# cartographer-project/point_cloud_viewer

Measured on AMD Instinct MI355X. Metric: octree-build Mpoints/sec, higher is better.
Workload: dtype f64; 1 GPU; BASELINE config 2: 100 M Gaussian-cluster points (64 clusters, 1000 m cube, sigma 1-20 m), f64 SoA xyz + u8 rgb, resolution 1 mm, full build + LOD promotion; points_per_gpu=100000000, points_total=100000000, nodes=6073, parallelism=1 GPU

## Files before the change

point_cloud_viewer_amd/csrc/pcv_encode.hip:

```cpp
#include <algorithm>
#include <cstdlib>

#include "pcv_chain_dev.h"
#include "pcv_settle_dev.h"
#include "pcv_spec.h"

#ifndef PCV_KEEP_BRANCH
#define PCV_KEEP_BRANCH 0
#endif
#ifndef PCV_ENC_SEGMENTS
#define PCV_ENC_SEGMENTS 1
#endif

namespace {

__global__ __launch_bounds__(256) void leaf_encode_kernel(
    PcvLevels lv, const uint64_t* __restrict__ walk, uint64_t n, const double* __restrict__ x,
    const double* __restrict__ y, const double* __restrict__ z, PcvRouted routed, const uint8_t* __restrict__ color,
    uint32_t color_stride, const float* __restrict__ intensity, uint32_t* __restrict__ rank, uint4* __restrict__ payload,
    uint32_t* __restrict__ cx_hi, uint32_t* __restrict__ cy_hi, uint32_t* __restrict__ cz_hi,
    uint32_t* __restrict__ inten_bits) {
  const uint64_t i = (uint64_t)blockIdx.x * 256 + threadIdx.x;
  if (i >= n) return;
  uint64_t rec = walk[0];
// ... 355 lines not shown
                             : make_uint4((uint32_t)vx, (uint32_t)vy, (uint32_t)vz, rgb);
      }
    }
  }
  tid = wave * 64 + (int)pcv_lane_again();
  if (stage) {
    uint32_t rgb[2];
#pragma unroll
    for (int h = 0; h < 2; ++h) {
      const uint32_t t = (uint32_t)(h * BLOCK + tid);
      rgb[h] = (!(DIAG & 1) && t < here) ? pcv_load_rgb(color + (base + t) * color_stride, base + t + 1 < n) : 0u;
    }
    __syncthreads();
#pragma unroll
    for (int h = 0; h < 2; ++h) {
      const uint32_t t = (uint32_t)(h * BLOCK + tid);
      if (t < here) {
        const uint2 q = opay[t];
        __builtin_nontemporal_store(okey[t] | (rgb[h] >> 16), &rank[base + t]);
        __builtin_nontemporal_store(((uint64_t)(q.y | ((rgb[h] & 0xffffu) << 16)) << 32) | q.x, reinterpret_cast<uint64_t*>(payload) + base + t);
      }
    }
  }
  if (inten_bits) {
#pragma unroll
    for (int h = 0; h < 2; ++h) {
      const uint32_t t = (uint32_t)(h * BLOCK + tid);
      if (t < here) inten_bits[base + t] = __float_as_uint(intensity[base + t]);
    }
  }
}
#undef CP_WALK_GUARDED
#undef CP_WALK_TAME
#undef CP_CODE_LOOP
#undef CP_LOOP
#undef CP_BITS
#undef CP_KEEP_STEP
#undef CP_WALK_AT


constexpr int kHistBins = 16384;
constexpr int kHistBinsRows = 32768;
__global__ __launch_bounds__(1024) void rank_hist_kernel(const uint32_t* __restrict__ rank, uint64_t n, uint64_t chunk,
                                                          uint32_t bin_base, uint32_t nbins, uint32_t* __restrict__ counts,
                                                          int shift ,
                                                          uint32_t* __restrict__ rows ,
                                                          uint32_t row_stride) {
  extern __shared__ uint32_t hist[];
  for (uint32_t b = threadIdx.x; b < nbins; b += 1024) hist[b] = 0;
  __syncthreads();
  const uint64_t begin = (uint64_t)blockIdx.x * chunk;
  uint64_t end = begin + chunk;
  if (end > n) end = n;
  for (uint64_t i = begin + (uint64_t)threadIdx.x * 4; i < end; i += 4096) {
    if (i + 4 <= end) {
      const uint4 v = *reinterpret_cast<const uint4*>(rank + i);
      const uint32_t r[4] = {(v.x >> shift) - bin_base, (v.y >> shift) - bin_base, (v.z >> shift) - bin_base,
                             (v.w >> shift) - bin_base};
#pragma unroll
      for (int k = 0; k < 4; ++k)
        if (r[k] < nbins) atomicAdd(&hist[r[k]], 1u);
    } else {
      for (uint64_t j = i; j < end; ++j) {
        const uint32_t r = (rank[j] >> shift) - bin_base;
        if (r < nbins) atomicAdd(&hist[r], 1u);
      }
    }
  }
  __syncthreads();
  for (uint32_t b = threadIdx.x; b < nbins; b += 1024) {
    const uint32_t v = hist[b];
    if (v) atomicAdd(&counts[bin_base + b], v);
    if (rows) rows[(uint64_t)blockIdx.x * row_stride + bin_base + b] = v;
  }
}

struct alignas(16) PcvContRange {
  uint32_t from_level, to_level, pad0, pad1;
  double mn[3];
  double pad2;
};
static_assert(sizeof(PcvContRange) == 48, "continue range");
__device__ __forceinline__ void pcv_continue_codes(const PcvLevels& lv, const PcvContRange& rg, uint32_t& cx, uint32_t& cy, uint32_t& cz) {
  const int from = (int)rg.from_level, to = (int)rg.to_level;
  const uint32_t fe = lv.enc[from], te = lv.enc[to];
  double mx = rg.mn[0], my = rg.mn[1], mz = rg.mn[2];
  const double e = lv.edge[from];
  double px = pcv_decode_coord(fe, cx, mx, e), py = pcv_decode_coord(fe, cy, my, e), pz = pcv_decode_coord(fe, cz, mz, e);
  double vx = 0, vy = 0, vz = 0;
  for (int L = from + 1; L <= to; ++L)
    (void)pcv_chain_level<true>(lv.enc[L], lv.edge[L - 1], lv.edge[L], PcvRecip{lv.inv_edge[L], lv.inv_edge_lo[L]}, px, py, pz, mx, my,
                                mz, vx, vy, vz);
  cx = (uint32_t)pcv_val_to_code(te, vx);
  cy = (uint32_t)pcv_val_to_code(te, vy);
  cz = (uint32_t)pcv_val_to_code(te, vz);
}
template <bool kCompact>
__global__ __launch_bounds__(256) void spec_continue_kernel(PcvLevels lv, const PcvContRange* __restrict__ ranges,
                                                             const PcvSettleItem* __restrict__ items, uint4* __restrict__ payload,
                                                             uint4* __restrict__ wide ) {
  const PcvSettleItem it = items[blockIdx.x];
  const PcvContRange rg = ranges[it.rank];
  const uint32_t fe = lv.enc[rg.from_level], te = lv.enc[rg.to_level];
  uint2* __restrict__ pay2 = reinterpret_cast<uint2*>(payload);
  for (uint32_t s = it.begin + threadIdx.x; s < it.end; s += 256) {
    uint4 p = make_uint4(0, 0, 0, 0);
    uint2 q = make_uint2(0, 0);
// ... 472 lines not shown
```

point_cloud_viewer_amd/csrc/pcv_internal.h:

```cpp
#pragma once
#include <hip/hip_runtime.h>
#include <stdint.h>

#include <condition_variable>
#include <functional>
#include <map>
#include <mutex>
#include <string>
#include <thread>
#include <vector>

#include "../../include/pcv_hip.h"
#include "pcv_levels.h"
#include "pcv_sort_plan.h"
#include "pcv_spec.h"

#define PCV_HIP_CHECK(ctx, expr)                                                                   \
  do {                                                                                             \
    hipError_t _e = (expr);                                                                        \
    if (_e != hipSuccess) return (ctx)->fail(PCV_E_HIP, std::string(#expr) + ": " + hipGetErrorString(_e)); \
  } while (0)

struct PcvHostPool {
  std::vector<std::thread> threads;
// ... 343 lines not shown
  uint32_t* dst = nullptr;
  uint64_t n = 0, chunk = 0;
  int shift = 0, nbits = 0;
  const uint32_t *hist = nullptr, *totals = nullptr;
  const void* vec_in = nullptr;
  void* vec_out = nullptr;
  const uint32_t* plane_in = nullptr;
  uint32_t* plane_out = nullptr;
  const uint32_t* map = nullptr;
  uint32_t map_entries = 0;
  const void* ranges = nullptr;
  const uint32_t* order = nullptr;
  const uint8_t* color_in = nullptr;
  uint32_t color_stride = 3;
};
void pcv_sort_launch_rec12(pcv_ctx* ctx, const PcvSortRec12Args& a);
void pcv_sort_launch_scan(pcv_ctx* ctx, uint32_t* hist, int groups, uint32_t* totals);
void pcv_sort_generic_passes_u32(pcv_ctx* ctx, const PcvSortPlan& plan, int first, uint32_t* keys_a, uint32_t* keys_b,
                                 PcvSortPayload* payload, void* scratch, const uint32_t* map, uint32_t map_entries);

struct PcvNodeTableDev {
  uint32_t capacity;
  uint64_t* prefix;
  uint64_t* prefix_lo;
  uint32_t* lo;
  uint32_t* hi;
  uint32_t* parent;
  uint32_t* first_child;
  uint8_t* level;
  uint8_t* child_mask;
  uint8_t* open;
  uint32_t* bounds;
  uint32_t max_open = 0;
  uint32_t* counters;
};
struct PcvPackedNode {
  uint64_t prefix;
  uint32_t lo, hi, first_child;
  uint8_t level, child_mask, open, pad;
};
static_assert(sizeof(PcvPackedNode) == 24, "packed node");
constexpr size_t kPcvPackHeader = 256;
void pcv_launch_pack_node_table(pcv_ctx* ctx, const PcvNodeTableDev& t, void* packed );
size_t pcv_sample_count_scratch_words(uint32_t capacity, uint32_t max_open, int nlevels);
void pcv_launch_sample_tree_counts(pcv_ctx* ctx, const PcvNodeTableDev& t, const uint64_t* keys, uint32_t n, const PcvLevels& lv,
                                   double resolution, uint32_t max_points_per_node, uint32_t force_split_level1_mask, uint32_t* scratch,
                                   uint32_t saturate_above );
void pcv_launch_spec_tree(pcv_ctx* ctx, const PcvNodeTableDev& t, double upper, uint32_t force_mask, uint32_t* ord, uint32_t* walk,
                          uint32_t* sparent, uint8_t* slevel, uint32_t* info, uint32_t* pool_ctr );
int pcv_launch_spec_sample_tree(pcv_ctx* ctx, const uint64_t* sorted_keys, uint32_t ns, const PcvLevels& lv, double resolution, uint32_t thr,
                                double upper, uint32_t force_mask, uint64_t* list, uint32_t list_cap, uint32_t* ctr, uint32_t* walk,
                                uint32_t* sparent, uint8_t* slevel, uint32_t* info, uint32_t* pool_ctr);
void pcv_launch_spec_resolve(pcv_ctx* ctx, const PcvLevels& lv, double resolution, uint32_t cap, uint32_t force_mask, const uint32_t* walk,
                             const uint8_t* slevel, uint32_t tn, uint32_t* counts, uint32_t* nst, uint32_t* base, uint32_t* map,
                             uint32_t* out);
void pcv_launch_node_split(pcv_ctx* ctx, const PcvNodeTableDev& t, const void* sorted_keys, bool keys32, uint32_t n,
                           const PcvLevels& lv, double resolution, uint32_t max_points_per_node,
                           uint32_t force_split_level1_mask, const uint64_t* sorted_lo = nullptr);
void pcv_launch_chain_keys_deep(pcv_ctx* ctx, const PcvLevels& lv, uint64_t n, const double* x, const double* y,
                                const double* z, const PcvRouted& routed, uint32_t* const words[4]);
void pcv_launch_combine_words(pcv_ctx* ctx, uint64_t n, const uint32_t* const words[4], uint64_t* hi, uint64_t* lo);

struct PcvWalkTables {
  uint32_t num_nodes;
  const uint64_t* walk;
};
void pcv_launch_leaf_encode(pcv_ctx* ctx, const PcvLevels& lv, const PcvWalkTables& wt, uint64_t n, const double* x,
                            const double* y, const double* z, const PcvRouted& routed, const uint8_t* color,
                            uint32_t color_stride, const float* intensity, uint32_t* rank, void* payload ,
                            uint32_t* cx_hi,
                            uint32_t* cy_hi, uint32_t* cz_hi, uint32_t* inten_bits);

void pcv_launch_spec_encode(pcv_ctx* ctx, const PcvLevels& lv, const uint32_t* walk, uint64_t n, const double* x,
                            const double* y, const double* z, const PcvRouted& routed, const uint8_t* color,
                            uint32_t color_stride, const float* intensity, uint32_t* rank, void* payload ,
                            uint32_t* inten_bits, uint8_t* depth_grid, void* wide, uint32_t* pool_ctr, const uint32_t* tree_info,
                            bool color_late = false ,
                            uint32_t* zero = nullptr ,
                            size_t zero_words = 0);
void pcv_launch_join_color(pcv_ctx* ctx, uint64_t n, const uint8_t* color, uint32_t color_stride, uint32_t* keys, void* payload_uint2);
constexpr uint32_t kPcvPoolRegions = 1024;
inline uint64_t pcv_pool_region_entries(uint64_t n) { return (((n + 1023) / 1024 + kPcvPoolRegions - 1) / kPcvPoolRegions) * 1024; }
size_t pcv_spec_depth_grid_bytes();
void pcv_launch_rank_hist(pcv_ctx* ctx, const uint32_t* rank, uint64_t n, uint32_t num_bins, uint32_t* counts ,
                          int shift = 0);
uint32_t pcv_rank_hist_max_bins();
void pcv_launch_rank_hist_rows(pcv_ctx* ctx, const uint32_t* rank, uint64_t n, uint32_t num_bins, uint32_t* counts ,
                               int shift, int groups, uint64_t chunk, uint32_t* rows );
void pcv_sort_rec12_geometry(uint64_t n, int* groups, uint64_t* chunk);
size_t pcv_cont_range_bytes();
void pcv_fill_cont_range(void* dst, uint32_t from_level, uint32_t to_level, const double mn[3]);
void pcv_launch_spec_continue(pcv_ctx* ctx, const PcvLevels& lv, const void* ranges, const PcvSettleItem* items, uint32_t num_items,
                              void* sorted_payload, void* wide = nullptr);
void pcv_launch_spec_replay(pcv_ctx* ctx, const PcvLevels& lv, const void* ranges, uint32_t num_ranges, uint32_t total,
                            const double* x, const double* y, const double* z, const PcvRouted& routed, void* sorted_payload,
                            void* wide = nullptr, uint32_t pool_cap = 0 );

struct alignas(16) PcvNodeRec {
  uint32_t lo;
  uint32_t parent;
  uint32_t child_off;
  uint32_t enc;
  uint64_t xyz_off;
  uint64_t point_off;
  double mn[3];
  double edge;
  double inv_edge;
// ... 59 lines not shown
```

point_cloud_viewer_amd/csrc/pcv_single_chain.hip:

```cpp
#include <algorithm>
#include <cmath>
#include <cstring>

#include "pcv_build_state.h"
#include "pcv_internal.h"
#include "pcv_spec.h"
#include "pcv_tables.h"

static bool pcv_settle_in_sort() { return pcv_switches().settle_in_sort && pcv_switches().settle_by_leaf; }

int pcv_queue_record_sort(pcv_ctx* ctx, PcvBuild* bs, pcv_octree* t, const PcvWalkTables* wt, uint32_t num_leaves, bool wide) {
  PcvScratch& sc = bs->sc;
  DevPoints& d = bs->d;
  PcvLevels& lv = bs->lv;
  const uint64_t n = bs->n;
  int rc;
  uint32_t* rank_a = (uint32_t*)bs->keys_a;
  uint32_t* rank_b = (uint32_t*)bs->keys_b;
  const bool compact = bs->spec_wide != nullptr;
  uint4 *pay_a = (uint4*)bs->spec_payload, *pay_b;
  if (compact) {
    uint2* b2;
    if ((rc = sc.get(&b2, n))) return rc;
    pay_b = (uint4*)b2;
// ... 287 lines not shown

  PCV_HIP_CHECK(ctx, hipStreamWaitEvent(ctx->side, ctx->side_fork, 0));
  PCV_HIP_CHECK(ctx, hipMemcpyAsync(hs, s.d_info, 16, hipMemcpyDeviceToHost, ctx->side));
  PCV_HIP_CHECK(ctx, hipMemcpyAsync(hs + kHostWalk, s.d_walk, first * 4, hipMemcpyDeviceToHost, ctx->side));
  PCV_HIP_CHECK(ctx, hipMemcpyAsync(hs + kHostParent, s.d_sparent, first * 4, hipMemcpyDeviceToHost, ctx->side));
  PCV_HIP_CHECK(ctx, hipMemcpyAsync(hs + kHostLevel, s.d_slevel, first, hipMemcpyDeviceToHost, ctx->side));
  PCV_HIP_CHECK(ctx, hipEventRecord(ctx->spec_ev, ctx->side));

  return read_mirror(s, out);
}

static int count_and_queue_sort(SingleChain& s) {
  pcv_ctx* ctx = s.ctx;
  PcvBuild* bs = s.bs;
  PcvScratch& sc = bs->sc;
  const PcvLevels& lv = bs->lv;
  const PcvSpecTree& tree = s.tree;
  const uint64_t n = bs->n;
  int rc;
  ctx->stage_begin(PCV_STAGE_NODE_SPLIT);
  bs->spec_rows = nullptr;
  if (pcv_switches().sort_rows && s.compact && tree.num_leaves <= pcv_rank_hist_max_bins()) {
    int sgroups;
    uint64_t schunk;
    pcv_sort_rec12_geometry(n, &sgroups, &schunk);
    uint32_t* rows = nullptr;
    if (sc.get(&rows, (size_t)sgroups * tree.num_leaves) == PCV_OK) {
      pcv_launch_rank_hist_rows(ctx, s.rank, n, tree.num_leaves, s.d_counts, 8, sgroups, schunk, rows);
      bs->spec_rows = rows;
    }
  }
  if (!bs->spec_rows) pcv_launch_rank_hist(ctx, s.rank, n, tree.num_leaves, s.d_counts, s.compact ? 8 : 0);
  PCV_HIP_CHECK(ctx, hipGetLastError());
  if ((rc = ctx->pinned_spec_reserve((size_t)tree.num_leaves * 8 + 512 + kPcvPoolRegions * 4))) return rc;
  uint8_t* hp = (uint8_t*)ctx->pinned_spec;
  s.h_pool = (uint32_t*)hp;
  s.h_counts = s.h_pool + kPcvPoolRegions;
  if (ctx->side_begin() != PCV_OK) return ctx->fail(PCV_E_HIP, "single-chain build: side stream");
  PCV_HIP_CHECK(ctx, hipMemcpyAsync(s.h_pool, s.d_pool_ctr, ((size_t)kPcvPoolRegions + tree.num_leaves) * 4, hipMemcpyDeviceToHost, ctx->side));
  PCV_HIP_CHECK(ctx, hipEventRecord(ctx->spec_ev, ctx->side));
  bs->spec_wide = s.wide;
  bs->wide_levels = s.wide_levels;
  bs->spec_map_dev = s.d_map;
  bs->spec_map_entries = tree.num_leaves;
  bs->spec = true;
  bs->spec_payload = s.payload;
  bs->fix_ranges.clear();
  uint32_t *d_nst, *d_base, *d_out;
  const uint32_t tn = (uint32_t)tree.prefix.size();
  if ((rc = sc.get(&d_nst, tn)) || (rc = sc.get(&d_base, tn))) return rc;
  d_out = (uint32_t*)(ctx->mailbox_dev + kPcvMailboxResolve);
  ctx->mailbox[kPcvMailboxResolve] = ~0ull;
  __atomic_thread_fence(__ATOMIC_SEQ_CST);
  pcv_launch_spec_resolve(ctx, lv, s.params->resolution, s.sp.cap, s.sp.force_mask, s.d_walk, s.d_slevel, tn, s.d_counts, d_nst, d_base, s.d_map, d_out);
  PCV_HIP_CHECK(ctx, hipGetLastError());
  bs->resolve_on_device = true;
  ctx->stage_end(PCV_STAGE_NODE_SPLIT);
  const uint32_t predicted_leaves = (uint32_t)std::count(tree.inner.begin(), tree.inner.end(), (uint8_t)0);
  return pcv_queue_record_sort(ctx, bs, s.t, nullptr, predicted_leaves, false);
}

static int settle_verdict(SingleChain& s, PcvTrueTree* tt, bool* used) {
  pcv_ctx* ctx = s.ctx;
  PcvBuild* bs = s.bs;
  pcv_octree* t = s.t;
  const PcvSpecTree& tree = s.tree;
  int rc;
  PCV_HIP_CHECK(ctx, hipEventSynchronize(ctx->spec_ev));
  const PcvSpecStatus resolved = pcv_spec_resolve(s.sp, tree, s.h_counts, tt);
  if (resolved != PCV_SPEC_OK) {
    bs->drop_single_chain(s.payload, s.wide);
    return PCV_OK;
  }
  if (s.wide) {
    uint64_t replay_slots = 0, used_entries = 0, most = 0;
    for (uint32_t k : tt->fix_nodes) replay_slots += tt->hi[k] - tt->lo[k];
    for (uint32_t r = 0; r < kPcvPoolRegions; ++r) {
      used_entries += s.h_pool[r];
      most = std::max<uint64_t>(most, s.h_pool[r]);
    }
    if (most + (replay_slots + kPcvPoolRegions - 1) / kPcvPoolRegions > s.pool_cap) {
      bs->drop_single_chain(s.payload, s.wide);
      return PCV_OK;
    }
    t->wide_pool_entries = used_entries;
  }
  bs->resolve_host_leaves = tt->num_leaves;
  bs->resolve_check_map = (s.params->flags & PCV_BUILD_CHECK_RESOLVE) != 0;
  if (bs->resolve_check_map) {
    bs->resolve_host_map = tt->spec_map;
    bs->resolve_host_inner = tree.inner;
  }
  if (tt->prefix.size() > (size_t)s.nt.capacity) return ctx->fail(PCV_E_OOM, "node table capacity exceeded");
  bs->cont_nodes = tt->cont_nodes;
  bs->cont_from = tt->cont_from;
  for (uint32_t k : tt->fix_nodes) bs->fix_ranges.push_back({tt->lo[k], tt->hi[k] - tt->lo[k], (uint32_t)tt->level[k]});
  if (!bs->sort_second.pending && (rc = pcv_queue_replay(ctx, bs))) return rc;
  ctx->stage_begin(PCV_STAGE_TABLE);
  t->spec_stats[0] = tree.prefix.size();
  t->spec_stats[1] = (uint64_t)std::count(tree.inner.begin(), tree.inner.end(), (uint8_t)0);
  t->spec_stats[2] = tt->kept_points;
  t->spec_stats[3] = tt->fix_points;
  t->spec_continued = tt->cont_points;
  *used = true;
  return PCV_OK;
}

// ... 21 lines not shown
```

point_cloud_viewer_amd/csrc/pcv_sort_rec12.hip:

```cpp
#include <algorithm>

#include "pcv_sort_dev.h"
#include "pcv_settle_dev.h"

#ifndef PCV_FUSE_DIAG
#define PCV_FUSE_DIAG 0
#endif

namespace {

template <int NW, int R>
struct DigitStateN {
  uint32_t whist[NW][R];
  uint32_t digit_base[R];
  uint32_t delta[R];
  uint32_t wave_tot[NW];
};

struct alignas(16) FuseLeaf {
  uint32_t lo, climb_base, flags;
  uint32_t count;
  uint64_t xyz_off;
  uint64_t point_off;
  double mn[3], edge, inv_edge, inv_edge_lo;
// ... 397 lines not shown


template <int BLOCK, int KPT, int R, int WPE, bool NT, int MAP = 0 , bool PL = false,
          bool WC = false>
__global__ __launch_bounds__(BLOCK, WPE) void downsweep_rec12_kernel(const uint32_t* __restrict__ keys_in,
                                                                     uint32_t* __restrict__ keys_out, uint64_t n, uint64_t chunk,
                                                                     int groups, int shift, int nbits,
                                                                     const uint32_t* __restrict__ offsets,
                                                                     const uint32_t* __restrict__ totals,
                                                                     const uint2* __restrict__ vec_in, uint2* __restrict__ vec_out,
                                                                     const uint32_t* __restrict__ gmap = nullptr, uint32_t map_entries = 0,
                                                                     const uint2* __restrict__ ranges = nullptr ,
                                                                     const uint32_t* __restrict__ order = nullptr ,
                                                                     const uint32_t* __restrict__ plane_in = nullptr,
                                                                     uint32_t* __restrict__ plane_out = nullptr,
                                                                     const uint8_t* __restrict__ color_in = nullptr ,
                                                                     uint32_t color_stride = 3) {
  downsweep_rec12_body<BLOCK, KPT, R, WPE, NT, MAP, PL, WC, false>(keys_in, keys_out, n, chunk, groups, shift, nbits, offsets, totals, vec_in,
                                                                  vec_out, gmap, map_entries, ranges, order, plane_in, plane_out, PcvSortFuse(),
                                                                  color_in, color_stride);
}
template <bool PL, int BLOCK = 1024, int R = 128>
__global__ __launch_bounds__(BLOCK, 4) void downsweep_settle_kernel(const uint32_t* __restrict__ keys_in, uint32_t* __restrict__ keys_out,
                                                                   uint64_t n, uint64_t chunk, int groups, int shift, int nbits,
                                                                   const uint32_t* __restrict__ offsets, const uint32_t* __restrict__ totals,
                                                                   const uint2* __restrict__ vec_in, uint2* __restrict__ vec_out,
                                                                   const uint2* __restrict__ ranges, const uint32_t* __restrict__ order,
                                                                   const uint32_t* __restrict__ plane_in, uint32_t* __restrict__ plane_out,
                                                                   PcvSortFuse fuse) {
  downsweep_rec12_body<BLOCK, 8, R, 4, false, 0, PL, false, true>(keys_in, keys_out, n, chunk, groups, shift, nbits, offsets, totals, vec_in,
                                                                   vec_out, nullptr, 0u, ranges, order, plane_in, plane_out, fuse);
}

__global__ __launch_bounds__(256) void hist_from_rows_kernel(const uint32_t* __restrict__ rows, uint32_t nbins,
                                                              const uint32_t* __restrict__ map, int rank_shift, uint32_t mask, int groups,
                                                              uint32_t* __restrict__ hist ) {
  __shared__ uint32_t h[kRadix];
  h[threadIdx.x] = 0;
  __syncthreads();
  const uint32_t* row = rows + (uint64_t)blockIdx.x * nbins;
  for (uint32_t b = threadIdx.x; b < nbins; b += 256) {
    const uint32_t c = row[b];
    if (c) atomicAdd(&h[((map[b] & PCV_SPEC_INDEX_MASK) >> rank_shift) & mask], c);
  }
  __syncthreads();
  hist[(uint64_t)threadIdx.x * groups + blockIdx.x] = threadIdx.x <= mask ? h[threadIdx.x] : 0u;
}

__global__ __launch_bounds__(256) void hist12_from_rows_kernel(const uint32_t* __restrict__ rows, uint32_t nbins,
                                                                const uint32_t* __restrict__ map, int nbits1, int nbits2, int groups,
                                                                uint32_t* __restrict__ hist1 ,
                                                                uint32_t* __restrict__ rows_true ,
                                                                int msd ) {
  extern __shared__ uint32_t tr[];
  const uint32_t D1 = 1u << nbits1, D2 = 1u << nbits2, TB = D1 * D2;
  const int sh1 = msd ? nbits2 : 0, sh2 = msd ? 0 : nbits1;
  const uint32_t rounds = TB > 32768u ? TB / 32768u : 1u, D1r = D1 / rounds, TBr = D1r * D2;
  const uint32_t* row = rows + (uint64_t)blockIdx.x * nbins;
  uint32_t* out = rows_true + (uint64_t)blockIdx.x * TB;
  hist1[(uint64_t)threadIdx.x * groups + blockIdx.x] = 0;
  for (uint32_t rd = 0; rd < rounds; ++rd) {
    const uint32_t d1_lo = rd * D1r;
    for (uint32_t i = threadIdx.x; i < TBr; i += 256) tr[i] = 0;
    __syncthreads();
    for (uint32_t b = threadIdx.x; b < nbins; b += 256) {
      const uint32_t c = row[b];
      if (c) {
        const uint32_t r = map[b] & PCV_SPEC_INDEX_MASK;
        const uint32_t d1 = ((r >> sh1) & (D1 - 1u)) - d1_lo;
        if (d1 < D1r) atomicAdd(&tr[d1 * D2 + ((r >> sh2) & (D2 - 1u))], c);
      }
    }
    __syncthreads();
    for (uint32_t i = threadIdx.x; i < TBr; i += 256) out[(uint64_t)d1_lo * D2 + i] = tr[i];
    if (threadIdx.x < D1r) {
      uint32_t s = 0;
      for (uint32_t d2 = 0; d2 < D2; ++d2) s += tr[threadIdx.x * D2 + ((d2 + threadIdx.x) & (D2 - 1u))];
      hist1[(uint64_t)(d1_lo + threadIdx.x) * groups + blockIdx.x] = s;
    }
    __syncthreads();
  }
}
__global__ __launch_bounds__(256) void pass2_layout_kernel(const uint32_t* __restrict__ rows_true, int nbits1, int nbits2, int groups,
                                                            int blocks, int gpb, const uint32_t* __restrict__ offsets1,
                                                            const uint32_t* __restrict__ totals1, int pieces,
                                                            uint32_t* __restrict__ hist2 , uint2* __restrict__ ranges,
                                                            uint32_t* __restrict__ order ) {
  __shared__ uint32_t part[4][256];
  const uint32_t D1 = 1u << nbits1, D2 = 1u << nbits2, TB = D1 * D2;
  const int k = blockIdx.x, d1 = k / blocks, blk = k % blocks;
  const int g_lo = blk * gpb, g_hi = (g_lo + gpb < groups) ? g_lo + gpb : groups;
  const uint32_t d2 = threadIdx.x & (D2 - 1u), lanes_per_g = 256u / D2, sub = threadIdx.x / D2;
  uint32_t s = 0;
  for (int g = g_lo + (int)sub; g < g_hi; g += (int)lanes_per_g) s += rows_true[(uint64_t)g * TB + (uint32_t)d1 * D2 + d2];
  (&part[0][0])[threadIdx.x] = s;
  __syncthreads();
  {
    uint32_t tot = 0;
    if (threadIdx.x < D2)
      for (uint32_t q = 0; q < lanes_per_g; ++q) tot += (&part[0][0])[q * D2 + threadIdx.x];
    hist2[(uint64_t)threadIdx.x * pieces + k] = tot;
  }
  if (threadIdx.x == 0) {
    uint32_t start = 0;
    for (int d = 0; d < d1; ++d) start += totals1[d];
    const uint32_t b = g_lo < groups ? start + offsets1[(uint64_t)d1 * groups + g_lo] : start + totals1[d1];
    const uint32_t e = g_hi < groups ? start + offsets1[(uint64_t)d1 * groups + g_hi] : start + totals1[d1];
    ranges[k] = make_uint2(b, e);
    const uint32_t mine = totals1[d1];
    uint32_t before = 0;
    for (int d = 0; d < (int)D1; ++d) {
      const uint32_t o = totals1[d];
      before += (o > mine || (o == mine && d < d1)) ? 1u : 0u;
    }
    order[before * (uint32_t)blocks + (uint32_t)blk] = (uint32_t)k;
  }
}

__global__ __launch_bounds__(256) void msd_offsets_kernel(uint32_t* __restrict__ hist2, int pieces, int blocks, int nbits2,
                                                           const uint32_t* __restrict__ totals1, uint32_t* __restrict__ totals2) {
  __shared__ uint32_t wave_tot[4];
  const int d1 = blockIdx.x;
  const uint32_t D2 = 1u << nbits2, total = D2 * (uint32_t)blocks;
  if (d1 == 0) totals2[threadIdx.x] = 0;
  uint32_t start = 0;
  for (int d = 0; d < d1; ++d) start += totals1[d];
  const uint32_t per = (total + 255u) / 256u;
// ... 219 lines not shown
```

point_cloud_viewer_amd/csrc/pcv_topology.hip:

```cpp
#include "pcv_internal.h"
#include "pcv_spec.h"

namespace {

enum { CNT_NODES = 0, CNT_ERROR = 1, CNT_LEVEL_START = 2, CNT_OPEN = 60  };

__device__ __forceinline__ uint32_t* pcv_split2_open_list(const PcvNodeTableDev& t, int which) {
  return t.bounds + (size_t)81 * t.max_open + (size_t)which * t.max_open;
}
__device__ __forceinline__ uint32_t* split2_mid_list(const PcvNodeTableDev& t) { return t.bounds + (size_t)83 * t.max_open; }

template <typename KeyT>
__device__ __forceinline__ uint32_t wave_lower_bound(const KeyT* __restrict__ keys, uint32_t lo, uint32_t hi,
                                                     KeyT target, int lane) {
  while (hi - lo > 64) {
    const uint32_t span = hi - lo;
    const uint32_t step = (span + 63) / 64;
    uint64_t idx = (uint64_t)lo + (uint64_t)(lane + 1) * step - 1;
    const bool in = idx < hi;
    const KeyT v = keys[in ? idx : (uint64_t)hi - 1];
    const uint64_t m = __ballot(in && v < target);
    const uint32_t cnt = __popcll(m);
    const uint64_t nlo = (uint64_t)lo + (uint64_t)cnt * step;
    const uint64_t nhi = (uint64_t)lo + (uint64_t)(cnt + 1) * step - 1;
// ... 741 lines not shown
    }
#pragma unroll
    for (uint32_t c = 0; c < 8; ++c) {
      walk[base + c] = rec[c];
      sparent[base + c] = id;
      slevel[base + c] = (uint8_t)(k + 1);
    }
  }
}

__global__ __launch_bounds__(1024) void spec_tree_build_kernel(uint64_t* __restrict__ list, uint32_t list_cap, const uint64_t* __restrict__ keys,
                                                                const uint32_t* __restrict__ ctr, uint32_t* __restrict__ walk,
                                                                uint32_t* __restrict__ sparent, uint8_t* __restrict__ slevel,
                                                                uint32_t* __restrict__ info, uint32_t* __restrict__ pool_ctr) {
  static_assert(kPcvPoolRegions <= 1024, "one counter per lane");
  extern __shared__ uint64_t lds_list[];
  __shared__ uint32_t lstart[PCV_MAX_KEY_LEVELS + 3];
  if (pool_ctr && threadIdx.x < kPcvPoolRegions) pool_ctr[threadIdx.x] = 0;
  const uint32_t m = ctr[0];
  uint32_t err = ctr[1];
  if (threadIdx.x < PCV_MAX_KEY_LEVELS + 3) lstart[threadIdx.x] = m;
  if (m > list_cap) {
    err |= 2u;
    if (threadIdx.x < 9) {
      walk[threadIdx.x] = threadIdx.x == 0 ? 1u : threadIdx.x | PCV_SPEC_LEAF;
      sparent[threadIdx.x] = threadIdx.x == 0 ? 0xffffffffu : 0u;
      slevel[threadIdx.x] = threadIdx.x == 0 ? 0 : 1;
    }
    if (threadIdx.x == 0) info[0] = 9u, info[1] = err, info[2] = m, info[3] = 0;
    return;
  }
  bool cand = false;
  if (m <= kSpecTreeLdsEntries) {
    for (uint32_t j = threadIdx.x; j < m; j += 1024) lds_list[j] = list[j];
    __syncthreads();
    spec_tree_build(lds_list, m, keys, walk, sparent, slevel, lstart);
    for (uint32_t j = 1 + threadIdx.x; j < m; j += 1024) cand = cand || (lds_list[j] >> 63);
  } else {
    __syncthreads();
    spec_tree_build(list, m, keys, walk, sparent, slevel, lstart);
    for (uint32_t j = 1 + threadIdx.x; j < m; j += 1024) cand = cand || (list[j] >> 63);
  }
  cand = __syncthreads_or(cand);
  if (threadIdx.x == 0) {
    info[0] = 1u + 8u * m;
    info[1] = err;
    info[2] = m;
    info[3] = cand ? 1u : 0u;
  }
}


template <bool kLds>
__global__ __launch_bounds__(1024) void spec_resolve_kernel(PcvLevels lv, double resolution, uint32_t cap, uint32_t force_mask,
                                                             const uint32_t* __restrict__ g_walk, const uint8_t* __restrict__ slevel,
                                                             uint32_t tn, uint32_t* __restrict__ g_cnt, uint32_t* __restrict__ g_nst,
                                                             uint32_t* __restrict__ g_base, uint32_t* __restrict__ map,
                                                             uint32_t* __restrict__ out ) {
  extern __shared__ uint32_t dyn[];
  __shared__ uint32_t lstart[PCV_MAX_KEY_LEVELS + 3];
  __shared__ uint32_t too_shallow;
  const uint32_t* walk = kLds ? dyn : g_walk;
  uint32_t* cnt = kLds ? dyn + tn : g_cnt;
  uint32_t* nst = kLds ? dyn + 2 * (size_t)tn : g_nst;
  uint32_t* base = kLds ? dyn + 3 * (size_t)tn : g_base;
  const uint32_t t = threadIdx.x;
  if (t < PCV_MAX_KEY_LEVELS + 3) lstart[t] = tn;
  if (t == 0) too_shallow = 0;
  if (kLds)
    for (uint32_t i = t; i < tn; i += 1024) {
      dyn[i] = g_walk[i];
      dyn[tn + i] = g_cnt[i];
    }
  __syncthreads();
  for (uint32_t i = t; i < tn; i += 1024)
    if (i == 0 || slevel[i] != slevel[i - 1]) lstart[slevel[i]] = i;
  __syncthreads();
  int maxl = 0;
  for (int l = 0; l <= PCV_MAX_KEY_LEVELS; ++l)
    if (lstart[l] < tn) maxl = l;
  const uint32_t l1_first = walk[0] & PCV_SPEC_INDEX_MASK;
  auto would_split = [&](uint32_t i, int level, uint32_t c) -> bool {
    if (level == 0) return true;
    if (level == 1 && ((force_mask >> ((i - l1_first) & 7u)) & 1u)) return true;
    return c > cap && lv.edge[level] > resolution;
  };
  constexpr uint32_t kLeavesMask = 0x0fffffffu;
  for (int L = maxl; L >= 0; --L) {
    const uint32_t b = lstart[L], e = lstart[L + 1];
    for (uint32_t i = b + t; i < e; i += 1024) {
      const uint32_t rec = walk[i];
      uint32_t c, nl;
      if (rec & PCV_SPEC_LEAF) {
        c = cnt[i];
        if (c > 0 && would_split(i, L, c)) atomicOr(&too_shallow, 1u);
        nl = c > 0 ? 1u : 0u;
      } else {
        const uint32_t first = rec & PCV_SPEC_INDEX_MASK;
        uint32_t cs[8], ns[8];
#pragma unroll
        for (int k = 0; k < 8; ++k) {
          cs[k] = cnt[first + k];
          ns[k] = nst[first + k] & kLeavesMask;
        }
        c = ((cs[0] + cs[1]) + (cs[2] + cs[3])) + ((cs[4] + cs[5]) + (cs[6] + cs[7]));
        cnt[i] = c;
        nl = would_split(i, L, c) ? ((ns[0] + ns[1]) + (ns[2] + ns[3])) + ((ns[4] + ns[5]) + (ns[6] + ns[7])) : (c > 0 ? 1u : 0u);
      }
      nst[i] = nl;
    }
    __syncthreads();
  }
  if (t == 0) {
    nst[0] = (nst[0] & kLeavesMask) | (1u << 28);
    base[0] = 0;
  }
  __syncthreads();
  for (int L = 0; L <= maxl; ++L) {
    const uint32_t b = lstart[L], e = lstart[L + 1];
    for (uint32_t i = b + t; i < e; i += 1024) {
      const uint32_t rec = walk[i];
      const uint32_t s = nst[i] >> 28;
      if (rec & PCV_SPEC_LEAF) {
        map[i] = (s & 3u) == 2u ? base[i] : 0u;
        continue;
      }
      const uint32_t first = rec & PCV_SPEC_INDEX_MASK;
      if ((s & 3u) == 1u) {
        uint32_t run = base[i];
        const uint32_t ca = ((s >> 2) & 1u) | ((rec & PCV_SPEC_CANDIDATE) ? 1u : 0u);
        uint32_t cs[8], ns[8], ws[8];
#pragma unroll
        for (int k = 0; k < 8; ++k) {
          cs[k] = cnt[first + k];
          ns[k] = nst[first + k] & kLeavesMask;
          ws[k] = walk[first + k];
        }
#pragma unroll
        for (int k = 0; k < 8; ++k) {
          const uint32_t ch = first + k;
          if (cs[k] == 0) {
            nst[ch] = ns[k];
          } else if (would_split(ch, L + 1, cs[k])) {
            nst[ch] = ns[k] | ((1u | (ca << 2)) << 28);
            base[ch] = run;
            run += ns[k];
          } else {
            const bool replay = !ca && !(ws[k] & PCV_SPEC_LEAF) && !(ws[k] & PCV_SPEC_CANDIDATE);
            nst[ch] = ns[k] | (2u << 28);
            base[ch] = run | (replay ? PCV_SPEC_MAP_REPLAY : 0u);
            run += 1;
          }
        }
      } else {
        const uint32_t v = base[i];
#pragma unroll
        for (int k = 0; k < 8; ++k) {
          nst[first + k] = (nst[first + k] & kLeavesMask) | (s << 28);
          base[first + k] = v;
        }
      }
    }
    __syncthreads();
  }
  if (t == 0) {
    out[0] = nst[0] & kLeavesMask;
    out[1] = too_shallow;
  }
}

}

void pcv_launch_spec_resolve(pcv_ctx* ctx, const PcvLevels& lv, double resolution, uint32_t cap, uint32_t force_mask, const uint32_t* walk,
                             const uint8_t* slevel, uint32_t tn, uint32_t* counts, uint32_t* nst, uint32_t* base, uint32_t* map,
                             uint32_t* out) {
  constexpr size_t kLdsBudget = 156 * 1024;
  static const bool lds_ok = hipFuncSetAttribute(reinterpret_cast<const void*>(&spec_resolve_kernel<true>),
                                                  hipFuncAttributeMaxDynamicSharedMemorySize, (int)kLdsBudget) == hipSuccess;
  const size_t need = (size_t)tn * 16;
  if (lds_ok && need <= kLdsBudget)
    hipLaunchKernelGGL((spec_resolve_kernel<true>), dim3(1), dim3(1024), need, ctx->stream, lv, resolution, cap, force_mask, walk, slevel, tn,
                       counts, nst, base, map, out);
  else
    hipLaunchKernelGGL((spec_resolve_kernel<false>), dim3(1), dim3(1024), 0, ctx->stream, lv, resolution, cap, force_mask, walk, slevel, tn,
                       counts, nst, base, map, out);
}

void pcv_launch_spec_tree(pcv_ctx* ctx, const PcvNodeTableDev& t, double upper, uint32_t force_mask, uint32_t* ord, uint32_t* walk,
                          uint32_t* sparent, uint8_t* slevel, uint32_t* info, uint32_t* pool_ctr) {
  hipLaunchKernelGGL(spec_tree_scan_kernel, dim3(1), dim3(1024), 0, ctx->stream, t, ord, info, pool_ctr);
  hipLaunchKernelGGL(spec_tree_emit_kernel, dim3(64), dim3(256), 0, ctx->stream, t, ord, upper, force_mask, walk, sparent, slevel,
                     info);
}

int pcv_launch_spec_sample_tree(pcv_ctx* ctx, const uint64_t* sorted_keys, uint32_t ns, const PcvLevels& lv, double resolution, uint32_t thr,
                                double upper, uint32_t force_mask, uint64_t* list, uint32_t list_cap, uint32_t* ctr, uint32_t* walk,
                                uint32_t* sparent, uint8_t* slevel, uint32_t* info, uint32_t* pool_ctr) {
  if (ns == 0 || lv.nlevels < 1 || lv.nlevels > PCV_MAX_KEY_LEVELS) return ctx->fail(PCV_E_INVALID, "sample tree: levels");
  static const bool lds_ok = hipFuncSetAttribute(reinterpret_cast<const void*>(&spec_tree_build_kernel),
                                                  hipFuncAttributeMaxDynamicSharedMemorySize,
                                                  (int)(kSpecTreeLdsEntries * sizeof(uint64_t))) == hipSuccess;
  if (!lds_ok) return ctx->fail(PCV_E_HIP, "sample tree: LDS");
  uint32_t edge_ok = 0;
  for (int k = 1; k <= lv.nlevels; ++k)
    if (lv.edge[k] > resolution) edge_ok |= 1u << k;
  const double uf = std::floor(upper);
  const uint32_t upper_floor = uf <= 0.0 ? 0u : (uf >= 4294967295.0 ? 0xffffffffu : (uint32_t)uf);
  {
    PcvProf prof(ctx, PCV_K_SPLIT_SEARCH);
    hipLaunchKernelGGL(spec_sample_open_kernel, dim3((ns + 255u) / 256u), dim3(256), 0, ctx->stream, sorted_keys, ns, (int)lv.nlevels,
                       edge_ok, thr, upper_floor, force_mask, list, list_cap, ctr);
  }
  {
    PcvProf prof(ctx, PCV_K_SPLIT_ASSIGN);
    hipLaunchKernelGGL(spec_tree_build_kernel, dim3(1), dim3(1024), kSpecTreeLdsEntries * sizeof(uint64_t), ctx->stream, list, list_cap,
                       sorted_keys, ctr, walk, sparent, slevel, info, pool_ctr);
  }
  return PCV_OK;
}

#ifdef PCV_EXPERIMENTS
size_t pcv_sample_count_scratch_words(uint32_t capacity, uint32_t max_open, int nlevels) {
  const size_t groups = (size_t)(nlevels + 2) / 3;
  return groups * (size_t)max_open * (kSlotCounters + 512u) + 2 * (size_t)capacity;
}
void pcv_launch_sample_tree_counts(pcv_ctx* ctx, const PcvNodeTableDev& t, const uint64_t* keys, uint32_t n, const PcvLevels& lv,
                                   double resolution, uint32_t max_points_per_node, uint32_t force_split_level1_mask, uint32_t* scratch,
                                   uint32_t saturate_above) {
  hipStream_t s = ctx->stream;
  const int groups = (lv.nlevels + 2) / 3;
  SampleCountTables c;
  c.max_open = t.max_open;
  c.counts = scratch;
  c.maps = c.counts + (size_t)groups * c.max_open * kSlotCounters;
  c.nslot = c.maps + (size_t)groups * c.max_open * 512u;
  c.nq = c.nslot + t.capacity;
  hipLaunchKernelGGL(sample_tree_init_kernel, dim3(1), dim3(256), 0, s, t, n, c);
// ... 65 lines not shown
```

Before: 23950 Mpoints/s.

## Vectorize histogram and resolve memory accesses, precompute level starts on host

The rank histogram kernel now issues four nontemporal 128-bit loads per thread before doing its atomics. The transpose-histogram kernel zeroes and copies its shared-memory table with 128-bit accesses and reads its row with aligned 128-bit loads. The single-block spec-resolve kernel pads its LDS arrays so each group of eight children is 16-byte aligned and loads and stores them as two uint4, and stages walk and counts with vector loads. It also takes level start offsets computed on the host from the tree level array instead of scanning slevel on the device. The goal is fewer memory instructions and less serial setup on small latency-bound kernels, at the cost of extra host work over tn nodes and some added alignment-dependent code paths.

```diff
diff --git a/point_cloud_viewer_amd/csrc/pcv_encode.hip b/point_cloud_viewer_amd/csrc/pcv_encode.hip
--- a/point_cloud_viewer_amd/csrc/pcv_encode.hip
+++ b/point_cloud_viewer_amd/csrc/pcv_encode.hip
@@ -431,7 +431,22 @@
   const uint64_t begin = (uint64_t)blockIdx.x * chunk;
   uint64_t end = begin + chunk;
   if (end > n) end = n;
-  for (uint64_t i = begin + (uint64_t)threadIdx.x * 4; i < end; i += 4096) {
+  uint64_t i = begin + (uint64_t)threadIdx.x * 4;
+  typedef uint32_t u4v __attribute__((ext_vector_type(4)));
+  constexpr int kLoads = 4;
+  for (; i + (kLoads - 1) * 4096 + 4 <= end; i += kLoads * 4096) {
+    u4v v[kLoads];
+#pragma unroll
+    for (int u = 0; u < kLoads; ++u) v[u] = __builtin_nontemporal_load(reinterpret_cast<const u4v*>(rank + i + u * 4096));
+#pragma unroll
+    for (int u = 0; u < kLoads; ++u)
+#pragma unroll
+      for (int k = 0; k < 4; ++k) {
+        const uint32_t r = (v[u][k] >> shift) - bin_base;
+        if (r < nbins) atomicAdd(&hist[r], 1u);
+      }
+  }
+  for (; i < end; i += 4096) {
     if (i + 4 <= end) {
       const uint4 v = *reinterpret_cast<const uint4*>(rank + i);
       const uint32_t r[4] = {(v.x >> shift) - bin_base, (v.y >> shift) - bin_base, (v.z >> shift) - bin_base,
diff --git a/point_cloud_viewer_amd/csrc/pcv_internal.h b/point_cloud_viewer_amd/csrc/pcv_internal.h
--- a/point_cloud_viewer_amd/csrc/pcv_internal.h
+++ b/point_cloud_viewer_amd/csrc/pcv_internal.h
@@ -419,7 +419,7 @@
                                 double upper, uint32_t force_mask, uint64_t* list, uint32_t list_cap, uint32_t* ctr, uint32_t* walk,
                                 uint32_t* sparent, uint8_t* slevel, uint32_t* info, uint32_t* pool_ctr);
 void pcv_launch_spec_resolve(pcv_ctx* ctx, const PcvLevels& lv, double resolution, uint32_t cap, uint32_t force_mask, const uint32_t* walk,
-                             const uint8_t* slevel, uint32_t tn, uint32_t* counts, uint32_t* nst, uint32_t* base, uint32_t* map,
+                             const uint8_t* host_level, uint32_t tn, uint32_t* counts, uint32_t* nst, uint32_t* base, uint32_t* map,
                              uint32_t* out);
 void pcv_launch_node_split(pcv_ctx* ctx, const PcvNodeTableDev& t, const void* sorted_keys, bool keys32, uint32_t n,
                            const PcvLevels& lv, double resolution, uint32_t max_points_per_node,
diff --git a/point_cloud_viewer_amd/csrc/pcv_single_chain.hip b/point_cloud_viewer_amd/csrc/pcv_single_chain.hip
--- a/point_cloud_viewer_amd/csrc/pcv_single_chain.hip
+++ b/point_cloud_viewer_amd/csrc/pcv_single_chain.hip
@@ -363,7 +363,7 @@
   d_out = (uint32_t*)(ctx->mailbox_dev + kPcvMailboxResolve);
   ctx->mailbox[kPcvMailboxResolve] = ~0ull;
   __atomic_thread_fence(__ATOMIC_SEQ_CST);
-  pcv_launch_spec_resolve(ctx, lv, s.params->resolution, s.sp.cap, s.sp.force_mask, s.d_walk, s.d_slevel, tn, s.d_counts, d_nst, d_base, s.d_map, d_out);
+  pcv_launch_spec_resolve(ctx, lv, s.params->resolution, s.sp.cap, s.sp.force_mask, s.d_walk, tree.level.data(), tn, s.d_counts, d_nst, d_base, s.d_map, d_out);
   PCV_HIP_CHECK(ctx, hipGetLastError());
   bs->resolve_on_device = true;
   ctx->stage_end(PCV_STAGE_NODE_SPLIT);
diff --git a/point_cloud_viewer_amd/csrc/pcv_sort_rec12.hip b/point_cloud_viewer_amd/csrc/pcv_sort_rec12.hip
--- a/point_cloud_viewer_amd/csrc/pcv_sort_rec12.hip
+++ b/point_cloud_viewer_amd/csrc/pcv_sort_rec12.hip
@@ -473,7 +473,7 @@
                                                                 uint32_t* __restrict__ hist1 ,
                                                                 uint32_t* __restrict__ rows_true ,
                                                                 int msd ) {
-  extern __shared__ uint32_t tr[];
+  extern __shared__ __align__(16) uint32_t tr[];
   const uint32_t D1 = 1u << nbits1, D2 = 1u << nbits2, TB = D1 * D2;
   const int sh1 = msd ? nbits2 : 0, sh2 = msd ? 0 : nbits1;
   const uint32_t rounds = TB > 32768u ? TB / 32768u : 1u, D1r = D1 / rounds, TBr = D1r * D2;
@@ -482,18 +482,38 @@
   hist1[(uint64_t)threadIdx.x * groups + blockIdx.x] = 0;
   for (uint32_t rd = 0; rd < rounds; ++rd) {
     const uint32_t d1_lo = rd * D1r;
-    for (uint32_t i = threadIdx.x; i < TBr; i += 256) tr[i] = 0;
+    const bool vec_tr = (TBr & 3u) == 0u;
+    if (vec_tr)
+      for (uint32_t i = threadIdx.x * 4; i < TBr; i += 1024) *reinterpret_cast<uint4*>(tr + i) = make_uint4(0u, 0u, 0u, 0u);
+    else
+      for (uint32_t i = threadIdx.x; i < TBr; i += 256) tr[i] = 0;
     __syncthreads();
-    for (uint32_t b = threadIdx.x; b < nbins; b += 256) {
-      const uint32_t c = row[b];
+    auto add = [&](uint32_t b, uint32_t c) {
       if (c) {
         const uint32_t r = map[b] & PCV_SPEC_INDEX_MASK;
         const uint32_t d1 = ((r >> sh1) & (D1 - 1u)) - d1_lo;
         if (d1 < D1r) atomicAdd(&tr[d1 * D2 + ((r >> sh2) & (D2 - 1u))], c);
       }
-    }
+    };
+    uint32_t head = (4u - (uint32_t)(((uint64_t)blockIdx.x * nbins) & 3u)) & 3u;
+    if (head > nbins) head = nbins;
+    const uint32_t nvec = (nbins - head) / 4u;
+    if (threadIdx.x < head) add(threadIdx.x, row[threadIdx.x]);
+    for (uint32_t v = threadIdx.x; v < nvec; v += 256) {
+      const uint32_t b = head + 4u * v;
+      const uint4 c = *reinterpret_cast<const uint4*>(row + b);
+      add(b, c.x);
+      add(b + 1u, c.y);
+      add(b + 2u, c.z);
+      add(b + 3u, c.w);
+    }
+    for (uint32_t b = head + 4u * nvec + threadIdx.x; b < nbins; b += 256) add(b, row[b]);
     __syncthreads();
-    for (uint32_t i = threadIdx.x; i < TBr; i += 256) out[(uint64_t)d1_lo * D2 + i] = tr[i];
+    if (vec_tr)
+      for (uint32_t i = threadIdx.x * 4; i < TBr; i += 1024)
+        *reinterpret_cast<uint4*>(out + (uint64_t)d1_lo * D2 + i) = *reinterpret_cast<const uint4*>(tr + i);
+    else
+      for (uint32_t i = threadIdx.x; i < TBr; i += 256) out[(uint64_t)d1_lo * D2 + i] = tr[i];
     if (threadIdx.x < D1r) {
       uint32_t s = 0;
       for (uint32_t d2 = 0; d2 < D2; ++d2) s += tr[threadIdx.x * D2 + ((d2 + threadIdx.x) & (D2 - 1u))];
diff --git a/point_cloud_viewer_amd/csrc/pcv_topology.hip b/point_cloud_viewer_amd/csrc/pcv_topology.hip
--- a/point_cloud_viewer_amd/csrc/pcv_topology.hip
+++ b/point_cloud_viewer_amd/csrc/pcv_topology.hip
@@ -817,33 +817,64 @@
 
 
 template <bool kLds>
+__device__ __forceinline__ void resolve_load8(const uint32_t* a, uint32_t first, uint32_t (&o)[8]) {
+  if (kLds && (first & 7u) == 1u) {
+    const uint4 lo = *reinterpret_cast<const uint4*>(a + first), hi = *reinterpret_cast<const uint4*>(a + first + 4);
+    o[0] = lo.x, o[1] = lo.y, o[2] = lo.z, o[3] = lo.w, o[4] = hi.x, o[5] = hi.y, o[6] = hi.z, o[7] = hi.w;
+  } else {
+#pragma unroll
+    for (int k = 0; k < 8; ++k) o[k] = a[first + k];
+  }
+}
+template <bool kLds>
+__device__ __forceinline__ void resolve_store8(uint32_t* a, uint32_t first, const uint32_t (&v)[8]) {
+  if (kLds && (first & 7u) == 1u) {
+    *reinterpret_cast<uint4*>(a + first) = make_uint4(v[0], v[1], v[2], v[3]);
+    *reinterpret_cast<uint4*>(a + first + 4) = make_uint4(v[4], v[5], v[6], v[7]);
+  } else {
+#pragma unroll
+    for (int k = 0; k < 8; ++k) a[first + k] = v[k];
+  }
+}
+__host__ __device__ inline size_t pcv_resolve_lds_stride(uint32_t tn) { return ((size_t)tn + 3 + 3) & ~(size_t)3; }
+struct PcvLevelStarts {
+  uint32_t at[PCV_MAX_KEY_LEVELS + 3];
+  int32_t maxl;
+};
+template <bool kLds>
 __global__ __launch_bounds__(1024) void spec_resolve_kernel(PcvLevels lv, double resolution, uint32_t cap, uint32_t force_mask,
-                                                             const uint32_t* __restrict__ g_walk, const uint8_t* __restrict__ slevel,
+                                                             const uint32_t* __restrict__ g_walk, PcvLevelStarts starts,
                                                              uint32_t tn, uint32_t* __restrict__ g_cnt, uint32_t* __restrict__ g_nst,
                                                              uint32_t* __restrict__ g_base, uint32_t* __restrict__ map,
                                                              uint32_t* __restrict__ out ) {
-  extern __shared__ uint32_t dyn[];
+  extern __shared__ __align__(16) uint32_t dyn[];
   __shared__ uint32_t lstart[PCV_MAX_KEY_LEVELS + 3];
   __shared__ uint32_t too_shallow;
-  const uint32_t* walk = kLds ? dyn : g_walk;
-  uint32_t* cnt = kLds ? dyn + tn : g_cnt;
-  uint32_t* nst = kLds ? dyn + 2 * (size_t)tn : g_nst;
-  uint32_t* base = kLds ? dyn + 3 * (size_t)tn : g_base;
+  const size_t ls = pcv_resolve_lds_stride(tn);
+  uint32_t* l_walk = dyn + 3;
+  const uint32_t* walk = kLds ? l_walk : g_walk;
+  uint32_t* cnt = kLds ? dyn + ls + 3 : g_cnt;
+  uint32_t* nst = kLds ? dyn + 2 * ls + 3 : g_nst;
+  uint32_t* base = kLds ? dyn + 3 * ls + 3 : g_base;
   const uint32_t t = threadIdx.x;
-  if (t < PCV_MAX_KEY_LEVELS + 3) lstart[t] = tn;
+  if (t < PCV_MAX_KEY_LEVELS + 3) lstart[t] = starts.at[t];
   if (t == 0) too_shallow = 0;
-  if (kLds)
-    for (uint32_t i = t; i < tn; i += 1024) {
-      dyn[i] = g_walk[i];
-      dyn[tn + i] = g_cnt[i];
-    }
-  __syncthreads();
-  for (uint32_t i = t; i < tn; i += 1024)
-    if (i == 0 || slevel[i] != slevel[i - 1]) lstart[slevel[i]] = i;
-  __syncthreads();
-  int maxl = 0;
-  for (int l = 0; l <= PCV_MAX_KEY_LEVELS; ++l)
-    if (lstart[l] < tn) maxl = l;
+  if (kLds) {
+    const uint32_t nvec = (((uintptr_t)g_walk | (uintptr_t)g_cnt) & 15) == 0 ? tn / 4u : 0u;
+    for (uint32_t v = t; v < nvec; v += 1024) {
+      const uint4 w = reinterpret_cast<const uint4*>(g_walk)[v];
+      const uint4 c = reinterpret_cast<const uint4*>(g_cnt)[v];
+      const uint32_t i = 4u * v;
+      l_walk[i] = w.x, l_walk[i + 1] = w.y, l_walk[i + 2] = w.z, l_walk[i + 3] = w.w;
+      cnt[i] = c.x, cnt[i + 1] = c.y, cnt[i + 2] = c.z, cnt[i + 3] = c.w;
+    }
+    for (uint32_t i = 4u * nvec + t; i < tn; i += 1024) {
+      l_walk[i] = g_walk[i];
+      cnt[i] = g_cnt[i];
+    }
+  }
+  __syncthreads();
+  const int maxl = starts.maxl;
   const uint32_t l1_first = walk[0] & PCV_SPEC_INDEX_MASK;
   auto would_split = [&](uint32_t i, int level, uint32_t c) -> bool {
     if (level == 0) return true;
@@ -863,11 +894,10 @@
       } else {
         const uint32_t first = rec & PCV_SPEC_INDEX_MASK;
         uint32_t cs[8], ns[8];
-#pragma unroll
-        for (int k = 0; k < 8; ++k) {
-          cs[k] = cnt[first + k];
-          ns[k] = nst[first + k] & kLeavesMask;
-        }
+        resolve_load8<kLds>(cnt, first, cs);
+        resolve_load8<kLds>(nst, first, ns);
+#pragma unroll
+        for (int k = 0; k < 8; ++k) ns[k] &= kLeavesMask;
         c = ((cs[0] + cs[1]) + (cs[2] + cs[3])) + ((cs[4] + cs[5]) + (cs[6] + cs[7]));
         cnt[i] = c;
         nl = would_split(i, L, c) ? ((ns[0] + ns[1]) + (ns[2] + ns[3])) + ((ns[4] + ns[5]) + (ns[6] + ns[7])) : (c > 0 ? 1u : 0u);
@@ -894,36 +924,39 @@
       if ((s & 3u) == 1u) {
         uint32_t run = base[i];
         const uint32_t ca = ((s >> 2) & 1u) | ((rec & PCV_SPEC_CANDIDATE) ? 1u : 0u);
-        uint32_t cs[8], ns[8], ws[8];
-#pragma unroll
-        for (int k = 0; k < 8; ++k) {
-          cs[k] = cnt[first + k];
-          ns[k] = nst[first + k] & kLeavesMask;
-          ws[k] = walk[first + k];
-        }
+        uint32_t cs[8], ns[8], ws[8], bs[8];
+        resolve_load8<kLds>(cnt, first, cs);
+        resolve_load8<kLds>(nst, first, ns);
+        resolve_load8<kLds>(walk, first, ws);
 #pragma unroll
         for (int k = 0; k < 8; ++k) {
           const uint32_t ch = first + k;
+          ns[k] &= kLeavesMask;
+          bs[k] = run;
           if (cs[k] == 0) {
-            nst[ch] = ns[k];
           } else if (would_split(ch, L + 1, cs[k])) {
-            nst[ch] = ns[k] | ((1u | (ca << 2)) << 28);
-            base[ch] = run;
             run += ns[k];
+            ns[k] |= (1u | (ca << 2)) << 28;
           } else {
             const bool replay = !ca && !(ws[k] & PCV_SPEC_LEAF) && !(ws[k] & PCV_SPEC_CANDIDATE);
-            nst[ch] = ns[k] | (2u << 28);
-            base[ch] = run | (replay ? PCV_SPEC_MAP_REPLAY : 0u);
+            ns[k] |= 2u << 28;
+            bs[k] |= replay ? PCV_SPEC_MAP_REPLAY : 0u;
             run += 1;
           }
         }
+        resolve_store8<kLds>(nst, first, ns);
+        resolve_store8<kLds>(base, first, bs);
       } else {
         const uint32_t v = base[i];
+        uint32_t ns[8], bs[8];
+        resolve_load8<kLds>(nst, first, ns);
 #pragma unroll
         for (int k = 0; k < 8; ++k) {
-          nst[first + k] = (nst[first + k] & kLeavesMask) | (s << 28);
-          base[first + k] = v;
+          ns[k] = (ns[k] & kLeavesMask) | (s << 28);
+          bs[k] = v;
         }
+        resolve_store8<kLds>(nst, first, ns);
+        resolve_store8<kLds>(base, first, bs);
       }
     }
     __syncthreads();
@@ -937,17 +970,24 @@
 }
 
 void pcv_launch_spec_resolve(pcv_ctx* ctx, const PcvLevels& lv, double resolution, uint32_t cap, uint32_t force_mask, const uint32_t* walk,
-                             const uint8_t* slevel, uint32_t tn, uint32_t* counts, uint32_t* nst, uint32_t* base, uint32_t* map,
+                             const uint8_t* host_level, uint32_t tn, uint32_t* counts, uint32_t* nst, uint32_t* base, uint32_t* map,
                              uint32_t* out) {
+  PcvLevelStarts starts;
+  for (uint32_t& a : starts.at) a = tn;
+  for (uint32_t i = 0; i < tn; ++i)
+    if ((i == 0 || host_level[i] != host_level[i - 1]) && host_level[i] <= PCV_MAX_KEY_LEVELS) starts.at[host_level[i]] = i;
+  starts.maxl = 0;
+  for (int l = 0; l <= PCV_MAX_KEY_LEVELS; ++l)
+    if (starts.at[l] < tn) starts.maxl = l;
   constexpr size_t kLdsBudget = 156 * 1024;
   static const bool lds_ok = hipFuncSetAttribute(reinterpret_cast<const void*>(&spec_resolve_kernel<true>),
                                                   hipFuncAttributeMaxDynamicSharedMemorySize, (int)kLdsBudget) == hipSuccess;
-  const size_t need = (size_t)tn * 16;
+  const size_t need = pcv_resolve_lds_stride(tn) * 16;
   if (lds_ok && need <= kLdsBudget)
-    hipLaunchKernelGGL((spec_resolve_kernel<true>), dim3(1), dim3(1024), need, ctx->stream, lv, resolution, cap, force_mask, walk, slevel, tn,
+    hipLaunchKernelGGL((spec_resolve_kernel<true>), dim3(1), dim3(1024), need, ctx->stream, lv, resolution, cap, force_mask, walk, starts, tn,
                        counts, nst, base, map, out);
   else
-    hipLaunchKernelGGL((spec_resolve_kernel<false>), dim3(1), dim3(1024), 0, ctx->stream, lv, resolution, cap, force_mask, walk, slevel, tn,
+    hipLaunchKernelGGL((spec_resolve_kernel<false>), dim3(1), dim3(1024), 0, ctx->stream, lv, resolution, cap, force_mask, walk, starts, tn,
                        counts, nst, base, map, out);
 }
 
```

Result: no change. 24180 Mpoints/s (median of 5 runs) (+0.9%).
